# google-research/weatherbenchX

Hardware: AMD Instinct MI355X
Metric: grid-point·metric evals/s (0.25° 721×1440×37L) at 1/2/4/8 GPUs; % HBM roofline (higher is better)
Workload: dtype f32+f64

## Files before the change

### weatherbenchx_amd/csrc/wbx_common.hpp

```cpp
#pragma once
#include <hip/hip_runtime.h>

#include <cstdarg>
#include <cstdint>
#include <cstdio>
#include <cstring>

#include "../../include/wbx.h"

struct wbx_ctx {
  int device = 0;
  int num_cus = 256;
  hipStream_t stream = nullptr;
  bool own_stream = false;
  hipEvent_t ev_start = nullptr;
  hipEvent_t ev_stop = nullptr;
  void* fft_state = nullptr;
  void* s2_scratch = nullptr;
  size_t s2_scratch_size = 0;
  void* aidm_scratch = nullptr;
  size_t aidm_scratch_size = 0;
  void* atoms_clean = nullptr;
  void* patch_counters = nullptr;
  size_t patch_counters_size = 0;
  uint32_t ens_queue_parity = 0;
  hipEvent_t* marks = nullptr;
  int marks_used = 0, marks_made = 0, marks_cap = 0;
};

namespace wbx {

char* last_error_buf();

inline int fail(int code, const char* fmt, ...) {
  va_list ap;
  va_start(ap, fmt);
  vsnprintf(last_error_buf(), 512, fmt, ap);
  va_end(ap);
  return code;
}

template <typename T>
__device__ __forceinline__ T ld_stream(const T* p) {
#ifdef WBX_LD_STREAM_PLAIN
  return *p;
#else
  return __builtin_nontemporal_load(p);
#endif
}

__device__ __forceinline__ const char* uniform_ptr(const char* p) {
  const uint64_t v = (uint64_t)p;
  const uint32_t lo = __builtin_amdgcn_readfirstlane((uint32_t)v), hi = __builtin_amdgcn_readfirstlane((uint32_t)(v >> 32));
  return (const char*)(((uint64_t)hi << 32) | lo);
}

template <typename T>
using global_ptr = const __attribute__((address_space(1))) T*;

template <typename T>
using const_ptr = const __attribute__((address_space(4))) T*;

static __constant__ int64_t wbx_zero_i64[1] = {0};
static __constant__ double wbx_one_f64[1] = {1.0};

__device__ __forceinline__ int64_t readlane64(int64_t v, int j) {
  const int lo = __builtin_amdgcn_readlane((int)(uint32_t)(uint64_t)v, j);
  const int hi = __builtin_amdgcn_readlane((int)(uint32_t)((uint64_t)v >> 32), j);
  return (int64_t)(((uint64_t)(uint32_t)hi << 32) | (uint32_t)lo);
}

__device__ __forceinline__ double wave_sum(double v) {
#pragma unroll
  for (int o = 32; o > 0; o >>= 1) v += __shfl_xor(v, o, 64);
  return v;
}

template <int CTRL, int ROW_MASK>
__device__ __forceinline__ double dpp_moved(double v) {
  const int lo = __builtin_amdgcn_update_dpp(0, __double2loint(v), CTRL, ROW_MASK, 0xf, true);
  const int hi = __builtin_amdgcn_update_dpp(0, __double2hiint(v), CTRL, ROW_MASK, 0xf, true);
  return __hiloint2double(hi, lo);
}

__device__ __forceinline__ double wave_sum_lane63(double v) {
  v += dpp_moved<0xB1, 0xf>(v);
  v += dpp_moved<0x4E, 0xf>(v);
  v += dpp_moved<0x124, 0xf>(v);
  v += dpp_moved<0x128, 0xf>(v);
  v += dpp_moved<0x142, 0xa>(v);
  v += dpp_moved<0x143, 0xc>(v);
  return v;
}

__device__ __forceinline__ double wave_sum_uniform(double v) {
  const double t = wave_sum_lane63(v);
  return __hiloint2double(__builtin_amdgcn_readlane(__double2hiint(t), 63), __builtin_amdgcn_readlane(__double2loint(t), 63));
}

}

#define WBX_HIP(expr)                                                                   \
  do {                                                                                  \
    hipError_t _e = (expr);                                                             \
    if (_e != hipSuccess)                                                               \
      return wbx::fail(WBX_ERR_HIP, "%s failed: %s (%s:%d)", #expr, hipGetErrorString(_e), \
                       __FILE__, __LINE__);                                             \
  } while (0)

#define WBX_REQUIRE(cond, ...)                                   \
  do {                                                           \
    if (!(cond)) return wbx::fail(WBX_ERR_INVALID, __VA_ARGS__); \
  } while (0)
```

### weatherbenchx_amd/csrc/wbx_ctx.hip

```cpp
#include <cstdlib>

#include <set>

#include "wbx_common.hpp"

namespace wbx {
char* last_error_buf() {
  static thread_local char buf[512] = "";
  return buf;
}
}

extern "C" int wbx_abi_version(void) { return WBX_ABI_VERSION; }

extern "C" const char* wbx_last_error(void) { return wbx::last_error_buf(); }

extern "C" int wbx_device_count(int* n_out) {
  WBX_REQUIRE(n_out != nullptr, "n_out is NULL");
  int n = 0;
  hipError_t e = hipGetDeviceCount(&n);
  if (e != hipSuccess) {
    *n_out = 0;
    return wbx::fail(WBX_ERR_NO_DEVICE, "hipGetDeviceCount: %s", hipGetErrorString(e));
  }
  *n_out = n;
  return 0;
}

extern "C" int wbx_ctx_create(int device_id, void* hip_stream, wbx_ctx** out) {
  WBX_REQUIRE(out != nullptr, "out is NULL");
  *out = nullptr;
  int n = 0;
  if (hipGetDeviceCount(&n) != hipSuccess || n <= 0)
    return wbx::fail(WBX_ERR_NO_DEVICE, "no HIP device visible (libwbx_hip has no CPU path)");
  WBX_REQUIRE(device_id >= 0 && device_id < n, "device_id %d out of range [0,%d)", device_id, n);
  WBX_HIP(hipSetDevice(device_id));
  wbx_ctx* c = new wbx_ctx();
  c->device = device_id;
  int cus = 0;
  if (hipDeviceGetAttribute(&cus, hipDeviceAttributeMultiprocessorCount, device_id) == hipSuccess && cus > 0) c->num_cus = cus;
  if (hip_stream) {
    c->stream = reinterpret_cast<hipStream_t>(hip_stream);
    c->own_stream = false;
  } else {
    hipError_t e = hipStreamCreateWithFlags(&c->stream, hipStreamNonBlocking);
    if (e != hipSuccess) {
      delete c;
      return wbx::fail(WBX_ERR_HIP, "hipStreamCreate: %s", hipGetErrorString(e));
    }
    c->own_stream = true;
  }
  if (hipEventCreate(&c->ev_start) != hipSuccess || hipEventCreate(&c->ev_stop) != hipSuccess) {
    delete c;
    return wbx::fail(WBX_ERR_HIP, "hipEventCreate failed");
  }
  *out = c;
  return 0;
}

namespace wbx {
void spectrum_release(wbx_ctx* ctx);
void spectrum_note_write(const void* dst, size_t bytes);
}

extern "C" int wbx_ctx_destroy(wbx_ctx* ctx) {
  if (!ctx) return 0;
  (void)hipSetDevice(ctx->device);
  (void)hipStreamSynchronize(ctx->stream);
  wbx::spectrum_release(ctx);
  if (ctx->s2_scratch) (void)hipFree(ctx->s2_scratch);
  if (ctx->aidm_scratch) (void)hipFree(ctx->aidm_scratch);
  if (ctx->patch_counters) (void)hipFree(ctx->patch_counters);
  delete static_cast<std::set<const void*>*>(ctx->atoms_clean);
  if (ctx->ev_start) (void)hipEventDestroy(ctx->ev_start);
  if (ctx->ev_stop) (void)hipEventDestroy(ctx->ev_stop);
  for (int i = 0; i < ctx->marks_made; ++i) (void)hipEventDestroy(ctx->marks[i]);
  free(ctx->marks);
  if (ctx->own_stream && ctx->stream) (void)hipStreamDestroy(ctx->stream);
  delete ctx;
  return 0;
}

extern "C" int wbx_ctx_synchronize(wbx_ctx* ctx) {
  WBX_REQUIRE(ctx != nullptr, "ctx is NULL");
  WBX_HIP(hipStreamSynchronize(ctx->stream));
  return 0;
}

extern "C" int wbx_ctx_device_name(wbx_ctx* ctx, char* buf, size_t buflen) {
  WBX_REQUIRE(ctx != nullptr && buf != nullptr && buflen > 0, "bad arguments");
  hipDeviceProp_t prop;
  WBX_HIP(hipGetDeviceProperties(&prop, ctx->device));
  snprintf(buf, buflen, "%s|%s|cus=%d", prop.name, prop.gcnArchName, prop.multiProcessorCount);
  return 0;
}

extern "C" int wbx_malloc(wbx_ctx* ctx, size_t bytes, void** dptr_out) {
  WBX_REQUIRE(ctx != nullptr && dptr_out != nullptr, "bad arguments");
  *dptr_out = nullptr;
  if (bytes == 0) return 0;
  WBX_HIP(hipSetDevice(ctx->device));
  WBX_HIP(hipMalloc(dptr_out, bytes));
  return 0;
}

extern "C" int wbx_free(wbx_ctx* ctx, void* dptr) {
  WBX_REQUIRE(ctx != nullptr, "ctx is NULL");
  if (!dptr) return 0;
  WBX_HIP(hipSetDevice(ctx->device));
  WBX_HIP(hipStreamSynchronize(ctx->stream));
  {
    hipDeviceptr_t base = nullptr;
    size_t size = 0;
    if (hipMemGetAddressRange(&base, &size, dptr) != hipSuccess) {
      (void)hipGetLastError();
      size = 1;
    }
    wbx::spectrum_note_write(dptr, size);
  }
  WBX_HIP(hipFree(dptr));
  return 0;
}

extern "C" int wbx_memcpy_h2d(wbx_ctx* ctx, void* dptr, const void* h_src, size_t bytes) {
  WBX_REQUIRE(ctx != nullptr, "ctx is NULL");
  if (bytes == 0) return 0;
  WBX_REQUIRE(dptr != nullptr && h_src != nullptr, "NULL pointer");
  WBX_HIP(hipSetDevice(ctx->device));
  wbx::spectrum_note_write(dptr, bytes);
  WBX_HIP(hipMemcpyAsync(dptr, h_src, bytes, hipMemcpyHostToDevice, ctx->stream));
  WBX_HIP(hipStreamSynchronize(ctx->stream));
  return 0;
}

extern "C" int wbx_memcpy_d2h(wbx_ctx* ctx, void* h_dst, const void* dptr, size_t bytes) {
  WBX_REQUIRE(ctx != nullptr, "ctx is NULL");
  if (bytes == 0) return 0;
  WBX_REQUIRE(dptr != nullptr && h_dst != nullptr, "NULL pointer");
  WBX_HIP(hipSetDevice(ctx->device));
  WBX_HIP(hipMemcpyAsync(h_dst, dptr, bytes, hipMemcpyDeviceToHost, ctx->stream));
  WBX_HIP(hipStreamSynchronize(ctx->stream));
  return 0;
}

extern "C" int wbx_host_alloc(wbx_ctx* ctx, size_t bytes, void** h_out) {
  WBX_REQUIRE(ctx != nullptr && h_out != nullptr, "NULL argument");
  WBX_HIP(hipSetDevice(ctx->device));
  WBX_HIP(hipHostMalloc(h_out, bytes ? bytes : 8, hipHostMallocDefault));
  return 0;
}

extern "C" int wbx_host_free(wbx_ctx* ctx, void* h_ptr) {
  WBX_REQUIRE(ctx != nullptr, "ctx is NULL");
  if (h_ptr) WBX_HIP(hipHostFree(h_ptr));
  return 0;
}

extern "C" int wbx_memcpy_d2h_async(wbx_ctx* ctx, void* h_pinned, const void* dptr, size_t bytes) {
  WBX_REQUIRE(ctx != nullptr, "ctx is NULL");
  if (bytes == 0) return 0;
  WBX_REQUIRE(dptr != nullptr && h_pinned != nullptr, "NULL pointer");
  WBX_HIP(hipSetDevice(ctx->device));
  WBX_HIP(hipMemcpyAsync(h_pinned, dptr, bytes, hipMemcpyDeviceToHost, ctx->stream));
  return 0;
}

struct wbx_fence {
  hipEvent_t ev;
};

extern "C" int wbx_fence_create(wbx_ctx* ctx, wbx_fence** out) {
  WBX_REQUIRE(ctx != nullptr && out != nullptr, "NULL argument");
  WBX_HIP(hipSetDevice(ctx->device));
  wbx_fence* f = new wbx_fence;
  hipError_t e = hipEventCreateWithFlags(&f->ev, hipEventDisableTiming);
  if (e != hipSuccess) {
    delete f;
    WBX_HIP(e);
  }
  *out = f;
  return 0;
}

extern "C" int wbx_fence_record(wbx_ctx* ctx, wbx_fence* f) {
  WBX_REQUIRE(ctx != nullptr && f != nullptr, "NULL argument");
  WBX_HIP(hipEventRecord(f->ev, ctx->stream));
  return 0;
}

extern "C" int wbx_fence_wait(wbx_fence* f) {
  WBX_REQUIRE(f != nullptr, "fence is NULL");
  WBX_HIP(hipEventSynchronize(f->ev));
  return 0;
}

extern "C" int wbx_ctx_wait_fence(wbx_ctx* ctx, wbx_fence* f) {
  WBX_REQUIRE(ctx != nullptr && f != nullptr, "NULL argument");
  WBX_HIP(hipStreamWaitEvent(ctx->stream, f->ev, 0));
  return 0;
}

extern "C" int wbx_fence_destroy(wbx_fence* f) {
  if (f) {
    (void)hipEventDestroy(f->ev);
    delete f;
  }
  return 0;
}

extern "C" int wbx_memset(wbx_ctx* ctx, void* dptr, int value, size_t bytes) {
  WBX_REQUIRE(ctx != nullptr, "ctx is NULL");
  if (bytes == 0) return 0;
  WBX_REQUIRE(dptr != nullptr, "NULL pointer");
  wbx::spectrum_note_write(dptr, bytes);
  WBX_HIP(hipMemsetAsync(dptr, value, bytes, ctx->stream));
  return 0;
}

extern "C" int wbx_timer_start(wbx_ctx* ctx) {
  WBX_REQUIRE(ctx != nullptr, "ctx is NULL");
  WBX_HIP(hipEventRecord(ctx->ev_start, ctx->stream));
  return 0;
}

extern "C" int wbx_mark(wbx_ctx* ctx, int* index_out) {
  WBX_REQUIRE(ctx != nullptr && index_out != nullptr, "bad arguments");
// ... 77 lines not shown
```

### weatherbenchx_amd/csrc/wbx_ens.hip

```cpp
#include "wbx_ens_atoms.hpp"
#include "wbx_ens_impl.hpp"

namespace wbx {

static int ens_common(wbx_ctx* ctx, const wbx_s1_plan* plan, int dtype, int M, int64_t member_stride, int algo,
                      const void* p, const void* t, const uint8_t* mask, double* out, bool map, int lane) {
  WBX_REQUIRE(ctx != nullptr, "ctx is NULL");
  if (int rc = check_plan(plan)) return rc;
  WBX_REQUIRE(plan->vec == 1, "ensemble kernels use vec=1");
  if (plan->flags & WBX_FLAG_MASKED) WBX_REQUIRE(mask != nullptr, "WBX_FLAG_MASKED set but mask is NULL");
  WBX_REQUIRE(M >= 1, "ensemble size must be >= 1 (got %d)", M);
  WBX_REQUIRE(algo == WBX_ENS_SORT || algo == WBX_ENS_PAIRWISE || (algo == WBX_ENS_DIAG_LOADONLY && (M == 50 || M == 51)) ||
                  (algo == WBX_ENS_DIAG_PAIRWISE_LDS && M == 51),
              "unknown ensemble algorithm %d", algo);
  const bool empty = plan->nkey * plan->ndepth * plan->nx == 0;
  WBX_REQUIRE(empty || (p != nullptr && t != nullptr), "predictions/targets pointer is NULL");
  WBX_REQUIRE(out != nullptr || plan->nkey == 0, "output pointer is NULL");
  WBX_HIP(hipSetDevice(ctx->device));
  S1Args a;
  fill_args(plan, a);
  a.in[0] = p;
  a.in[1] = t;
  a.in[3] = mask;
  a.out = out;
  a.M = M;
  a.mstride = member_stride;
  a.lane = lane;
  if (dtype == WBX_F64) return launch_ens_op<EnsOpGeneric<double>>(ctx, plan, a, map);
  WBX_REQUIRE(dtype == WBX_F32, "unknown dtype %d", dtype);
  if (plan->flags & WBX_FLAG_SKIPNA_ENS) {
    static const bool generic = getenv("WBX_ENS_SKIPNA_GENERIC") && atoi(getenv("WBX_ENS_SKIPNA_GENERIC")) != 0;
    if (generic || M > 64) return launch_ens_op<EnsOpGeneric<float>>(ctx, plan, a, map);
    algo = WBX_ENS_SKIPNA_SORT;
  }
  if (M == 51) return launch_ens_m51(ctx, plan, a, algo, map);
  if (M == 50) return launch_ens_m50(ctx, plan, a, algo, map);
  if (M <= 4) return launch_ens_m4(ctx, plan, a, algo, map);
  if (M <= 8) return launch_ens_m8(ctx, plan, a, algo, map);
  if (M <= 16) return launch_ens_m16(ctx, plan, a, algo, map);
  if (M <= 32) return launch_ens_m32(ctx, plan, a, algo, map);
  if (M <= 64) return launch_ens_m64(ctx, plan, a, algo, map);
  return launch_ens_op<EnsOpGeneric<float>>(ctx, plan, a, map);
}

}

extern "C" int wbx_ens_partial(wbx_ctx* ctx, const wbx_s1_plan* plan, int dtype, int M, int64_t member_stride,
                               int algo, const void* p, const void* t, const uint8_t* mask, double* partial_out) {
  return wbx::ens_common(ctx, plan, dtype, M, member_stride, algo, p, t, mask, partial_out, false, 0);
}

extern "C" int wbx_ens_map(wbx_ctx* ctx, const wbx_s1_plan* plan, int dtype, int M, int64_t member_stride, int algo,
                           int lane, const void* p, const void* t, double* out) {
  if (lane < 0 || lane >= WBX_ENS_LANES) return wbx::fail(WBX_ERR_INVALID, "ensemble lane %d out of range", lane);
  return wbx::ens_common(ctx, plan, dtype, M, member_stride, algo, p, t, nullptr, out, true, lane);
}

namespace wbx {

static int ens_binned_geometry(const wbx_s1_plan* plan, int64_t nA, int64_t nBk, int64_t nBr, int32_t w_on_x, BinnedArgs& g) {
  if (int rc = check_plan(plan)) return rc;
  WBX_REQUIRE(nA >= 1 && nBk >= 1 && nBr >= 1 && plan->nx >= 1 && plan->ndepth >= 1, "empty geometry");
  patch_geometry(g, nA * nBk, nBk, nBr, (w_on_x & WBX_BINNED_W_ON_X) ? plan->nx : 1, plan->ndepth, plan->nx, ens_atoms_rows(), ens_atoms_taper());
  return 0;
}

}

extern "C" int wbx_ens_binned_atoms_size(const wbx_s1_plan* plan, int64_t nA, int64_t nBk, int64_t nBr, int32_t w_on_x,
                                         int64_t* bytes_out) {
  using namespace wbx;
  WBX_REQUIRE(bytes_out != nullptr, "bytes_out is NULL");
  BinnedArgs g;
  if (int rc = ens_binned_geometry(plan, nA, nBk, nBr, w_on_x, g)) return rc;
  *bytes_out = (int64_t)atoms_carve(g, nullptr);
  return 0;
}

extern "C" int wbx_ens_binned_atoms(wbx_ctx* ctx, const wbx_s1_plan* plan, int64_t nA, int64_t nBk, int64_t nBr,
                                    int32_t w_on_x, const uint64_t* bits, void* atoms_out, int64_t* overflow_out) {
  using namespace wbx;
  WBX_REQUIRE(ctx != nullptr, "ctx is NULL");
  WBX_REQUIRE(bits != nullptr && atoms_out != nullptr, "NULL pointer");
  BinnedArgs g;
  if (int rc = ens_binned_geometry(plan, nA, nBk, nBr, w_on_x, g)) return rc;
  WBX_HIP(hipSetDevice(ctx->device));
  atoms_carve(g, atoms_out);
  if (int rc = atoms_launch(ctx, g, bits, plan->ndepth, plan->nx, true)) return rc;
  if (overflow_out) {
    const size_t n = (size_t)g.nBk * g.nrs * g.nxt;
    int32_t* host = (int32_t*)malloc(n * sizeof(int32_t));
    WBX_REQUIRE(host != nullptr, "out of host memory");
    hipError_t err = hipMemcpyAsync(host, g.nwords, n * sizeof(int32_t), hipMemcpyDeviceToHost, ctx->stream);
    if (err == hipSuccess) err = hipStreamSynchronize(ctx->stream);
    int64_t bad = 0;
    for (size_t i = 0; i < n && err == hipSuccess; ++i) bad += host[i] < 0;
    free(host);
    WBX_HIP(err);
    *overflow_out = bad;
  }
  return 0;
}

extern "C" int wbx_ens_binned(wbx_ctx* ctx, const wbx_s1_plan* plan, int dtype, int M, int64_t member_stride, int algo,
                              const void* p, const void* t, const uint8_t* mask, const double* wt, const uint64_t* bits,
                              int64_t nA, int64_t nBk, int64_t nBr, int32_t w_on_x, int32_t nbin, const void* atoms,
                              double* out) {
  using namespace wbx;
  WBX_REQUIRE(ctx != nullptr, "ctx is NULL");
  if (int rc = check_plan(plan)) return rc;
  WBX_REQUIRE(dtype == WBX_F32, "wbx_ens_binned takes float32 members (got dtype %d)", dtype);
  WBX_REQUIRE(algo == WBX_ENS_SORT, "wbx_ens_binned runs the rank form (WBX_ENS_SORT) only");
  WBX_REQUIRE(M >= 2 && M <= 64, "wbx_ens_binned handles 2..64 members (got %d)", M);
  WBX_REQUIRE(!(plan->flags & WBX_FLAG_SKIPNA_ENS), "wbx_ens_binned does not take skipna_ensemble (per-point member counts)");
  WBX_REQUIRE(nbin >= 1 && nbin <= 64, "wbx_ens_binned handles 1..64 bins (got %d)", nbin);
  WBX_REQUIRE(nA >= 0 && nBk >= 0 && nBr >= 0 && nA * nBk * nBr == plan->nkey, "nA*nBk*nBr must equal plan->nkey");
  WBX_REQUIRE((w_on_x & ~63) == 0 && (w_on_x & 6) != 6, "w_on_x: unknown or contradictory WBX_BINNED_* flags (%d)", w_on_x);
  WBX_REQUIRE(wt == nullptr || (w_on_x & (WBX_BINNED_WT_X_ONLY | WBX_BINNED_WT_ROW_ONLY)),
              "wbx_ens_binned takes factored weights only (WBX_BINNED_WT_X_ONLY / WBX_BINNED_WT_ROW_ONLY), or wt = NULL");
  WBX_REQUIRE(!(w_on_x & WBX_BINNED_WT_X_ONLY) || (w_on_x & WBX_BINNED_W_ON_X), "WBX_BINNED_WT_X_ONLY needs WBX_BINNED_W_ON_X");
  const bool twin_out = (plan->flags & WBX_FLAG_MASKED) && (w_on_x & WBX_BINNED_TWIN_MASK);
  const bool skipna = (plan->flags & WBX_FLAG_SKIPNA) != 0;
  const int64_t nout = nA * nBk * (skipna ? (twin_out ? 20 : 10) : (twin_out ? ENS_ATOMS_NOUT2 : ENS_ATOMS_NOUT)) * nbin;
  if (nout == 0) return 0;
  WBX_REQUIRE(out != nullptr, "out is NULL");
  WBX_HIP(hipSetDevice(ctx->device));
  if (nBr * plan->ndepth * plan->nx == 0) {
    if (!(w_on_x & WBX_BINNED_ACCUMULATE)) WBX_HIP(hipMemsetAsync(out, 0, (size_t)nout * sizeof(double), ctx->stream));
    return 0;
  }
  WBX_REQUIRE(p != nullptr && t != nullptr && bits != nullptr, "p/t/bits is NULL");
  if (plan->flags & WBX_FLAG_MASKED) {
    WBX_REQUIRE(mask != nullptr, "WBX_FLAG_MASKED set but mask is NULL");
    WBX_REQUIRE(w_on_x & WBX_BINNED_W_ON_X, "wbx_ens_binned with a validity mask needs W indexed per x (WBX_BINNED_W_ON_X)");
    WBX_REQUIRE(plan->xstride[3] >= 0, "the mask's x stride must be non-negative");
  }
  WBX_REQUIRE(plan->xstride[0] >= 0 && plan->xstride[1] >= 0 && (double)plan->nx * (double)plan->xstride[0] * 4.0 < 4294967296.0 &&
                  (double)plan->nx * (double)plan->xstride[1] * 4.0 < 4294967296.0,
              "x offsets of the members and of the targets must be non-negative and fit 32 bits");
  S1Args a;
  fill_args(plan, a);
  a.in[0] = p;
  a.in[1] = t;
  a.in[3] = mask;
  a.M = M;
  a.mstride = member_stride;
  EnsBinnedCall c;
  c.wt = wt;
  c.bits = bits;
  c.nA = nA;
  c.nBk = nBk;
  c.nBr = nBr;
  c.nj = (w_on_x & WBX_BINNED_W_ON_X) ? plan->nx : 1;
  c.nbin = nbin;
  c.w_on_x = w_on_x;
  c.prepared = atoms;
  c.out = out;
  if (M == 51) return launch_ens_atoms_m51(ctx, plan, a, c);
  if (M == 50) return launch_ens_atoms_m50(ctx, plan, a, c);
  if (M <= 4) return launch_ens_atoms_m4(ctx, plan, a, c);
  if (M <= 8) return launch_ens_atoms_m8(ctx, plan, a, c);
  if (M <= 16) return launch_ens_atoms_m16(ctx, plan, a, c);
  if (M <= 32) return launch_ens_atoms_m32(ctx, plan, a, c);
  return launch_ens_atoms_m64(ctx, plan, a, c);
}
```

### weatherbenchx_amd/csrc/wbx_ens_impl.hpp

```cpp
#pragma once
#include <cmath>
#include <cstdlib>

#include "wbx_s1.hpp"
#include "wbx_sortnet_gen.hpp"
#include "wbx_sortnet3_gen.hpp"

#ifndef WBX_ENS_MIN_WAVES
#define WBX_ENS_MIN_WAVES 1
#endif

#ifndef WBX_ENS_MIN_WAVES_PLAIN
#define WBX_ENS_MIN_WAVES_PLAIN WBX_ENS_MIN_WAVES
#endif
#ifndef WBX_ENS_SORTNET3
#define WBX_ENS_SORTNET3 1
#endif

#ifndef WBX_ENS_NOFALLBACK
#define WBX_ENS_NOFALLBACK 0
#endif
#ifndef WBX_ENS_STATS32
#define WBX_ENS_STATS32 1
#endif

namespace wbx {

constexpr int WBX_ENS_DIAG_LOADONLY = 99;
constexpr int WBX_ENS_DIAG_PAIRWISE_LDS = 98;
constexpr int WBX_ENS_SKIPNA_SORT = 97;

template <typename T>
struct EnsOpGeneric {
  static constexpr int NIN = 2;
  static constexpr int NLANE = WBX_ENS_LANES;
  static constexpr int NACC = WBX_ENS_LANES;
  static constexpr int XR_UNROLL = 1, XK_UNROLL = 1, MIN_WAVES = 1;

  __device__ __forceinline__ static void values(const S1Args& a, const int64_t (&ro)[WBX_MAX_INPUTS], int64_t x,
                                                double (&val)[NLANE]) {
    const int M = a.M;
    const T* pp = reinterpret_cast<const T*>(a.in[0]) + ro[0] + x * a.xstride[0];
    const double td = (double)(reinterpret_cast<const T*>(a.in[1])[ro[1] + x * a.xstride[1]]);
    const bool skip = a.flags & WBX_FLAG_SKIPNA_ENS;
    double se = 0.0, sq = 0.0, sabs = 0.0, pair_total = 0.0, x0 = 0.0;
    int n = 0;
    for (int i = 0; i < M; ++i) {
      const double xi = (double)pp[(int64_t)i * a.mstride];
      if (skip && xi != xi) continue;
      if (n == 0) x0 = xi;
      ++n;
      const double e = xi - x0;
      se += e;
      sq = fma(e, e, sq);
      sabs += fabs(xi - td);
      double row = 0.0;
      for (int j = 0; j < i; ++j) {
        const double xj = (double)pp[(int64_t)j * a.mstride];
        if (skip && xj != xj) continue;
        row += fabs(xi - xj);
      }
      pair_total += row;
    }
    const double dM = (double)n;
    const double fair = (a.flags & WBX_FLAG_FAIR) ? 1.0 : 0.0;
    const double mean_e = se / dM;
    const double mean_d = (x0 - td) + mean_e;
    const double var = (sq - se * mean_e) / (dM - 1.0);
    val[0] = sabs / dM;
    val[1] = 2.0 * pair_total / (dM * (dM - fair));
    val[2] = var;
    val[3] = mean_d * mean_d - var / dM;
    val[4] = mean_d * mean_d;
  }

  template <int V, bool XK>
  __device__ __forceinline__ static void accum(const S1Args& a, const int64_t (&ro)[WBX_MAX_INPUTS], int64_t x,
                                               double (&acc)[XK ? V : 1][NACC]) {
    static_assert(V == 1, "ensemble op is one point per lane");
    double val[NLANE];
    values(a, ro, x, val);
#pragma unroll
    for (int l = 0; l < NLANE; ++l) acc[0][l] += val[l];
  }
};

template <int MP, bool EXACT, int ALGO>
struct EnsOpF32 {
  static constexpr int NIN = 2;
  static constexpr int NLANE = WBX_ENS_LANES;
  static constexpr int NACC = WBX_ENS_LANES;
  static constexpr int XR_UNROLL = 1, XK_UNROLL = 1, MIN_WAVES = WBX_ENS_MIN_WAVES_PLAIN;

  struct Regs {
    float xm[MP];
    float t;
    float poison;
  };

  __device__ __forceinline__ static void load(const S1Args& a, const int64_t (&ro)[WBX_MAX_INPUTS], int64_t x, Regs& r) {
    const int M = EXACT ? MP : a.M;
    const float* pp = reinterpret_cast<const float*>(a.in[0]) + ro[0] + x * a.xstride[0];
    r.t = ld_stream(reinterpret_cast<const float*>(a.in[1]) + ro[1] + x * a.xstride[1]);
#pragma unroll
    for (int m = 0; m < MP; ++m) r.xm[m] = (EXACT || m < M) ? ld_stream(pp + (int64_t)m * a.mstride) : INFINITY;
  }

  __device__ __forceinline__ static void values(const S1Args& a, const int64_t (&ro)[WBX_MAX_INPUTS], int64_t x,
                                                double (&val)[NLANE]) {
    Regs r;
    load(a, ro, x, r);
    finish(a, ro, x, r, val);
  }

  template <bool FAST32 = false>
  __device__ __forceinline__ static bool compute(const S1Args& a, Regs& r, double (&val)[NLANE]) {
    const int M = EXACT ? MP : a.M;
    const double td = (double)r.t;
    float(&xm)[MP] = r.xm;

    if constexpr (ALGO == WBX_ENS_DIAG_LOADONLY) {
      float s = 0.f;
#pragma unroll
      for (int m = 0; m < MP; ++m)
        if (EXACT || m < M) s += xm[m];
      val[0] = (double)s - td;
      val[1] = val[2] = val[3] = val[4] = 0.0;
      return false;
    }
    double pair_total = 0.0;
    float poison = 0.f;
    int nvalid = 0;
    bool weird = false;
    float shift32 = 0.f;
    if constexpr (ALGO == WBX_ENS_SKIPNA_SORT) {
      const bool tfin32 = (r.t - r.t) == 0.f;
      shift32 = r.t;
      if (__builtin_amdgcn_ballot_w64(!tfin32)) {
        float lo = INFINITY;
#pragma unroll
        for (int m = 0; m < MP; ++m)
          if (EXACT || m < M) lo = fminf(lo, xm[m]);
        shift32 = tfin32 ? r.t : lo;
      }
#pragma unroll
      for (int m = 0; m < MP; ++m) {
        if (EXACT || m < M) {
          const float x = xm[m];
          const bool missing = x != x;
          nvalid += missing ? 0 : 1;
          xm[m] = missing ? shift32 : x;
        }
      }
      if constexpr (!EXACT) {
        float big = 0.f;
        int m = 0;
// ... 168 lines not shown
    const double mean_d = x0t + mean_e;
    const double var = (sq - se * mean_e) * inv_m1;
    double spread;
    if constexpr (ALGO == WBX_ENS_SORT) {
      spread = dot * spread_scale;
    } else {
      spread = pair_total * spread_scale;
    }
    if constexpr (ALGO == WBX_ENS_DIAG_PAIRWISE_LDS) {
      static_assert(EXACT && MP % 17 == 0, "the LDS-tiled diagnostic is instantiated for M = 51");
      constexpr int B = 17, NB = MP / B;
      __shared__ float tile[MP][64];
      float* col = &tile[0][threadIdx.x];
#pragma unroll
      for (int m = 0; m < MP; ++m) col[m * 64] = xm[m];
      asm volatile("" ::: "memory");
      double total = 0.0;
#pragma unroll
      for (int bi = 0; bi < NB; ++bi) {
        float xi[B];
#pragma unroll
        for (int k = 0; k < B; ++k) xi[k] = col[(bi * B + k) * 64];
#pragma unroll
        for (int k = 1; k < B; ++k) {
          float row = 0.f;
#pragma unroll
          for (int l = 0; l < k; ++l) row += fabsf(xi[k] - xi[l]);
          total += (double)row;
        }
#pragma unroll
        for (int bj = 0; bj < bi; ++bj) {
          float xj[B];
#pragma unroll
          for (int l = 0; l < B; ++l) xj[l] = col[(bj * B + l) * 64];
#pragma unroll
          for (int k = 0; k < B; ++k) {
            float row = 0.f;
#pragma unroll
            for (int l = 0; l < B; ++l) row += fabsf(xi[k] - xj[l]);
            total += (double)row;
          }
        }
      }
      spread = total * spread_scale;
    }
    val[0] = sabs * inv_m;
    val[1] = spread;
    val[2] = var;
    val[3] = mean_d * mean_d - var * inv_m;
    val[4] = mean_d * mean_d;
  }

  __device__ __forceinline__ static void stats32(const S1Args& a, float (&xm)[MP], const float t, const float poison,
                                                 double (&val)[NLANE]) {
    static_assert(EXACT, "fp32 chain sums are instantiated for the exact-M buckets");
    constexpr int K = 8, MID = MP / 2, NPAIR = MP / 2;
    const float c = xm[MID];
    float se[K], sq[K], sa[K], dt[K];
#pragma unroll
    for (int k = 0; k < K; ++k) se[k] = sq[k] = sa[k] = dt[k] = k == 0 ? poison : 0.f;
#pragma unroll
    for (int i = 0; i < NPAIR; ++i) {
      const int j = MP - 1 - i, k = i % K;
      const float ei = xm[i] - c, ej = xm[j] - c;
      se[k] += ei + ej;
      sq[k] = fmaf(ei, ei, sq[k]);
      sq[k] = fmaf(ej, ej, sq[k]);
      sa[k] += fabsf(xm[i] - t);
      sa[k] += fabsf(xm[j] - t);
      dt[k] = fmaf((float)(MP - 1 - 2 * i), xm[j] - xm[i], dt[k]);
    }
    if constexpr (MP & 1) {
      sa[NPAIR % K] += fabsf(c - t);
    } else {
    }
    auto fold = [](const float (&v)[K]) {
      return ((double)(v[0] + v[4]) + (double)(v[1] + v[5])) + ((double)(v[2] + v[6]) + (double)(v[3] + v[7]));
    };
    const double dse = fold(se), dsq = fold(sq), dsa = fold(sa), ddt = fold(dt);
    constexpr double dM = (double)MP;
    const double fair = (a.flags & WBX_FLAG_FAIR) ? 1.0 : 0.0;
    constexpr double inv_m = 1.0 / dM, inv_m1 = 1.0 / (dM - 1.0);
    const double spread_scale = 2.0 / (dM * (dM - fair));
    const double mean_e = dse * inv_m;
    const double mean_d = ((double)c - (double)t) + mean_e;
    const double var = (dsq - dse * mean_e) * inv_m1;
    val[0] = dsa * inv_m;
    val[1] = ddt * spread_scale;
    val[2] = var;
    val[3] = mean_d * mean_d - var * inv_m;
    val[4] = mean_d * mean_d;
  }

  template <int V, bool XK>
  __device__ __forceinline__ static void accum(const S1Args& a, const int64_t (&ro)[WBX_MAX_INPUTS], int64_t x,
                                               double (&acc)[XK ? V : 1][NACC]) {
    static_assert(V == 1, "ensemble op is one point per lane");
    double val[NLANE];
    values(a, ro, x, val);
#pragma unroll
    for (int l = 0; l < NLANE; ++l) acc[0][l] += val[l];
  }
};

template <class Core, bool SKIPNA>
struct EnsMasked {
  static constexpr int NIN = Core::NIN;
  static constexpr int NLANE = Core::NLANE;
  static constexpr int NACC = Core::NLANE + (SKIPNA ? Core::NLANE : 1);
  static constexpr int XR_UNROLL = 1, XK_UNROLL = 1, MIN_WAVES = WBX_ENS_MIN_WAVES;

  __device__ __forceinline__ static void values(const S1Args& a, const int64_t (&ro)[WBX_MAX_INPUTS], int64_t x,
                                                double (&val)[NLANE]) {
    Core::values(a, ro, x, val);
  }

  template <int V, bool XK>
  __device__ __forceinline__ static void accum(const S1Args& a, const int64_t (&ro)[WBX_MAX_INPUTS], int64_t x,
                                               double (&acc)[XK ? V : 1][NACC]) {
    static_assert(V == 1, "ensemble op is one point per lane");
    double val[NLANE];
    Core::values(a, ro, x, val);
    const bool valid =
        (a.flags & WBX_FLAG_MASKED) ? reinterpret_cast<const uint8_t*>(a.in[3])[ro[3] + x * a.xstride[3]] != 0 : true;
    if constexpr (!SKIPNA) {
#pragma unroll
      for (int l = 0; l < NLANE; ++l) acc[0][l] += valid ? val[l] : 0.0;
      acc[0][NLANE] += valid ? 1.0 : 0.0;
    } else {
#pragma unroll
      for (int l = 0; l < NLANE; ++l) {
        const bool ok = valid && !(val[l] != val[l]);
        acc[0][l] += ok ? val[l] : 0.0;
        acc[0][NLANE + l] += ok ? 1.0 : 0.0;
      }
    }
  }
};


#pragma clang diagnostic push
#pragma clang diagnostic ignored "-Winline-asm"
#ifndef WBX_ENS_PIPE_NLDS
#define WBX_ENS_PIPE_NLDS 50
#endif
#ifndef WBX_ENS_PIPE_WAVES
#define WBX_ENS_PIPE_WAVES 3
#endif
#ifndef WBX_ENS_PIPE_SKIPNA_WAVES
#define WBX_ENS_PIPE_SKIPNA_WAVES 3
#endif
template <int MP, bool EXACT, int ALGO, bool FLAT>
__global__ void __launch_bounds__(64, ALGO == WBX_ENS_SKIPNA_SORT ? WBX_ENS_PIPE_SKIPNA_WAVES : WBX_ENS_PIPE_WAVES)
ens_pipe_kernel(S1Args a, int R) {
  using Op = EnsOpF32<MP, EXACT, ALGO>;
  constexpr int NA = Op::NACC;
  constexpr int NLDS = MP < WBX_ENS_PIPE_NLDS ? MP : WBX_ENS_PIPE_NLDS;
  constexpr int NREG = MP - NLDS;
  __shared__ float stage[NLDS][64];
  const int lane = threadIdx.x;
  const int M = EXACT ? MP : a.M;
  const int64_t b = blockIdx.x;
  const int64_t key = b / a.nchunk;
  const int chunk = (int)(b - key * a.nchunk);
  const int64_t d0 = (int64_t)chunk * a.dchunk;
  const int64_t d1 = d0 + a.dchunk < a.D ? d0 + a.dchunk : a.D;
  const int nx = (int)a.nx;
  const uint32_t lds0 = (uint32_t)(uintptr_t)(__attribute__((address_space(3))) void*)&stage[0][0];
  const int64_t mstride_b = a.mstride * 4;

  int64_t kb[WBX_MAX_INPUTS], ro[WBX_MAX_INPUTS];
  key_bases<2>(a, key, kb);
  double acc[NA];
#pragma unroll
  for (int l = 0; l < NA; ++l) acc[l] = 0.0;

  int64_t d = d0, e0 = 0, e1 = 0, et = 0;
  int wm = 0;
  const int wstep = 64 % nx;
  auto open_segment = [&]() {
    if constexpr (FLAT) {
      const int64_t plane = d / R;
      const int64_t j0 = d - plane * R;
      const int64_t nj = d1 - d < R - j0 ? d1 - d : R - j0;
      row_bases<2>(a, kb, key, plane * R, ro);
      e0 = j0 * nx;
      e1 = (j0 + nj) * nx;
      et = e0 & ~(int64_t)63;
      wm = (int)((et + lane) % nx);
      d += nj;
    } else {
      row_bases<2>(a, kb, key, d, ro);
      e0 = 0;
      e1 = nx;
      et = 0;
      d += 1;
    }
  };

  float xn[NREG > 0 ? NREG : 1], tn = 0.f;
  double wn = 0.0;
  auto issue = [&]() {
    int64_t e = et + lane;
    e = e < e0 ? e0 : (e < e1 ? e : e1 - 1);
    const uint32_t voff = (uint32_t)e * (uint32_t)a.xstride[0] * 4u;
    const char* um = uniform_ptr(reinterpret_cast<const char*>(a.in[0]) + ro[0] * 4);
#pragma unroll
    for (int m = 0; m < NLDS; ++m) {
      if (EXACT || m < M)
        asm volatile("s_add_u32 m0, %2, %3\n\tglobal_load_lds_dword %0, %1 nt" ::"v"(voff), "s"(um), "s"(lds0), "i"(m * 256)
                     : "memory", "scc", "m0");
      um += mstride_b;
      asm volatile("" : "+s"(um));
    }
    const float* pr = reinterpret_cast<const float*>(a.in[0]) + ro[0] + e * a.xstride[0];
#pragma unroll
    for (int m = NLDS; m < MP; ++m) xn[m - NLDS] = (EXACT || m < M) ? ld_stream(pr + (int64_t)m * a.mstride) : INFINITY;
    tn = ld_stream(reinterpret_cast<const float*>(a.in[1]) + ro[1] + e * a.xstride[1]);
    if constexpr (FLAT) wn = a.xw[wm];
  };

  bool more = d < d1;
  if (more) {
    open_segment();
    issue();
  }
  while (more) {
    typename Op::Regs r;
    asm volatile("s_waitcnt vmcnt(0)" ::: "memory");
#pragma unroll
    for (int m = 0; m < NLDS; ++m) r.xm[m] = (EXACT || m < M) ? stage[m][lane] : INFINITY;
#pragma unroll
    for (int m = NLDS; m < MP; ++m) r.xm[m] = xn[m - NLDS];
    r.t = tn;
    const double wcur = wn;
    const int64_t ecur = et + lane;
    const bool valid = ecur >= e0 && ecur < e1;
    const int64_t xcur = ecur < e0 ? e0 : (ecur < e1 ? ecur : e1 - 1);
    int64_t rocur[WBX_MAX_INPUTS];
#pragma unroll
    for (int i = 0; i < WBX_MAX_INPUTS; ++i) rocur[i] = ro[i];
    const bool full = et >= e0 && et + 64 <= e1;
    et += 64;
    if (et >= e1) {
      more = d < d1;
      if (more) open_segment();
    } else if constexpr (FLAT) {
      wm += wstep;
      wm = wm >= nx ? wm - nx : wm;
    }
    asm volatile("s_waitcnt lgkmcnt(0)" ::: "memory");
    if (more) issue();
    double val[Op::NLANE];
    Op::template finish<true>(a, rocur, xcur, r, val);
    if constexpr (FLAT) {
      if (full) {
#pragma unroll
        for (int l = 0; l < NA; ++l) acc[l] = fma(val[l], wcur, acc[l]);
      } else {
#pragma unroll
        for (int l = 0; l < NA; ++l) acc[l] = fma(valid ? val[l] : 0.0, wcur, acc[l]);
      }
    } else if (full) {
#pragma unroll
      for (int l = 0; l < NA; ++l) acc[l] += val[l];
    } else {
#pragma unroll
      for (int l = 0; l < NA; ++l) acc[l] += valid ? val[l] : 0.0;
    }
  }
#pragma unroll
  for (int l = 0; l < NA; ++l) {
    const double v = wave_sum(acc[l]);
    if (lane == l) a.out[(key * a.nchunk + chunk) * NA + l] = v;
  }
}

#pragma clang diagnostic pop

inline bool ens_pipe_ok(const wbx_s1_plan* plan, const S1Args& a, bool skipna_ens = false) {
  static const bool off = getenv("WBX_ENS_PIPE") && atoi(getenv("WBX_ENS_PIPE")) == 0;
  static const bool off_skipna = getenv("WBX_ENS_PIPE_SKIPNA") && atoi(getenv("WBX_ENS_PIPE_SKIPNA")) == 0;
  if (off || (skipna_ens && off_skipna)) return false;
  if (plan->x_kept || plan->x_weights != nullptr || plan->block_threads != 64) return false;
  if (plan->flags & (WBX_FLAG_MASKED | WBX_FLAG_SKIPNA | (skipna_ens ? 0u : (unsigned)WBX_FLAG_SKIPNA_ENS))) return false;
  if (plan->nx <= 0 || plan->ndepth <= 0 || plan->nkey <= 0) return false;
  if (a.xstride[0] < 0 || a.xstride[1] < 0) return false;
  return (double)plan->nx * (double)a.xstride[0] * 4.0 < 4294967296.0;
}

inline bool ens_pipe_flat_ok(const wbx_s1_plan* plan, const S1Args& a) {
  static const bool off = getenv("WBX_ENS_PIPE") && atoi(getenv("WBX_ENS_PIPE")) == 0;
  if (off) return false;
  if (plan->x_kept || plan->x_weights == nullptr || plan->block_threads != 64 || plan->plane_rows <= 0) return false;
  if (plan->flags & (WBX_FLAG_MASKED | WBX_FLAG_SKIPNA | WBX_FLAG_SKIPNA_ENS)) return false;
  if (plan->nx <= 0 || plan->nx > WBX_XW_MAX || plan->ndepth <= 0 || plan->nkey <= 0 || plan->ndepth % plan->plane_rows != 0) return false;
  if (a.xstride[0] != 1 || a.xstride[1] != 1) return false;
  return (double)plan->nx * (double)plan->plane_rows * 4.0 < 4294967296.0;
}

template <int MP, bool EXACT, int ALGO, bool FLAT = false>
int launch_ens_pipe(wbx_ctx* ctx, const wbx_s1_plan* plan, S1Args& a) {
  const int64_t grid = plan->nkey * plan->nchunk;
  WBX_REQUIRE(grid < (int64_t)1 << 31, "grid too large (%lld blocks)", (long long)grid);
  hipLaunchKernelGGL((ens_pipe_kernel<MP, EXACT, ALGO, FLAT>), dim3((unsigned)grid), dim3(64), 0, ctx->stream, a,
                     FLAT ? plan->plane_rows : 0);
  WBX_HIP(hipGetLastError());
  return 0;
}

template <class Op>
int launch_ens_op(wbx_ctx* ctx, const wbx_s1_plan* plan, S1Args& a, bool map) {
  if (map) return launch_map<Op>(ctx, plan, a);
  if (plan->x_weights != nullptr) {
    WBX_REQUIRE(!(plan->flags & WBX_FLAG_SKIPNA_ENS), "flat x-weighted mode does not take skipna_ensemble");
    if (plan->flags & WBX_FLAG_SKIPNA) return launch_flat_weighted1<EnsMasked<Op, true>>(ctx, plan, a);
    if (plan->flags & WBX_FLAG_MASKED) return launch_flat_weighted1<EnsMasked<Op, false>>(ctx, plan, a);
    return launch_flat_weighted1<Op>(ctx, plan, a);
  }
  if (plan->flags & WBX_FLAG_SKIPNA) return launch_partial<EnsMasked<Op, true>, 1>(ctx, plan, a);
  if (plan->flags & WBX_FLAG_MASKED) return launch_partial<EnsMasked<Op, false>, 1>(ctx, plan, a);
  return launch_partial<Op, 1>(ctx, plan, a);
}

template <int MP, bool EXACT>
int launch_ens_bucket(wbx_ctx* ctx, const wbx_s1_plan* plan, S1Args& a, int algo, bool map) {
  if (!map && algo == WBX_ENS_SORT && ens_pipe_ok(plan, a)) return launch_ens_pipe<MP, EXACT, WBX_ENS_SORT>(ctx, plan, a);
  if (!map && algo == WBX_ENS_SORT && ens_pipe_flat_ok(plan, a)) return launch_ens_pipe<MP, EXACT, WBX_ENS_SORT, true>(ctx, plan, a);
  if (algo == WBX_ENS_SORT) return launch_ens_op<EnsOpF32<MP, EXACT, WBX_ENS_SORT>>(ctx, plan, a, map);
  if (algo == WBX_ENS_DIAG_LOADONLY) {
    if (!EXACT || map) return fail(WBX_ERR_INVALID, "the load-only diagnostic exists for the exact-M partial kernels only");
    return launch_partial<EnsOpF32<MP, EXACT, WBX_ENS_DIAG_LOADONLY>, 1>(ctx, plan, a);
  }
  if (algo == WBX_ENS_DIAG_PAIRWISE_LDS) {
    if constexpr (EXACT && MP == 51) {
      if (map || plan->x_weights != nullptr || (plan->flags & (WBX_FLAG_MASKED | WBX_FLAG_SKIPNA)) || plan->block_threads != 64)
        return fail(WBX_ERR_INVALID, "the LDS-tiled pair-form diagnostic exists for the plain partial kernels with one-wave blocks only");
      return launch_partial<EnsOpF32<MP, EXACT, WBX_ENS_DIAG_PAIRWISE_LDS>, 1>(ctx, plan, a);
    } else {
      return fail(WBX_ERR_INVALID, "the LDS-tiled pair-form diagnostic exists for M = 51 only");
    }
  }
  if (!map && algo == WBX_ENS_SKIPNA_SORT && ens_pipe_ok(plan, a, true)) return launch_ens_pipe<MP, EXACT, WBX_ENS_SKIPNA_SORT>(ctx, plan, a);
  if (algo == WBX_ENS_SKIPNA_SORT) return launch_ens_op<EnsOpF32<MP, EXACT, WBX_ENS_SKIPNA_SORT>>(ctx, plan, a, map);
  return launch_ens_op<EnsOpF32<MP, EXACT, WBX_ENS_PAIRWISE>>(ctx, plan, a, map);
}

int launch_ens_m4(wbx_ctx*, const wbx_s1_plan*, S1Args&, int, bool);
int launch_ens_m8(wbx_ctx*, const wbx_s1_plan*, S1Args&, int, bool);
int launch_ens_m16(wbx_ctx*, const wbx_s1_plan*, S1Args&, int, bool);
int launch_ens_m32(wbx_ctx*, const wbx_s1_plan*, S1Args&, int, bool);
int launch_ens_m64(wbx_ctx*, const wbx_s1_plan*, S1Args&, int, bool);
int launch_ens_m50(wbx_ctx*, const wbx_s1_plan*, S1Args&, int, bool);
int launch_ens_m51(wbx_ctx*, const wbx_s1_plan*, S1Args&, int, bool);

}
```

Measured before the change: 119.5 billion.

## Taper tail of ensemble pipe grid by splitting last blocks into pieces

Splits the final logical blocks of the ensemble pipe kernel into 2/4/8 sub-pieces sized from the number of blocks that can be resident at once. Each piece covers a slice of the tile range and writes a partial sum to scratch, and a small fixup kernel then adds the partials into the output. The goal is to cut the tail-wave imbalance where a few long blocks run alone at the end of the launch. The cost is an extra kernel launch, scratch traffic, occupancy queries cached per kernel, and extra index arithmetic in every block.

```diff
diff --git a/weatherbenchx_amd/csrc/wbx_common.hpp b/weatherbenchx_amd/csrc/wbx_common.hpp
--- a/weatherbenchx_amd/csrc/wbx_common.hpp
+++ b/weatherbenchx_amd/csrc/wbx_common.hpp
@@ -24,6 +24,10 @@
   void* patch_counters = nullptr;
   size_t patch_counters_size = 0;
   uint32_t ens_queue_parity = 0;
+  void* ens_taper_scratch = nullptr;
+  size_t ens_taper_scratch_size = 0;
+  int32_t ens_pipe_last[5] = {0, 0, 0, 0, 0};
+  void* ens_pipe_resident = nullptr;
   hipEvent_t* marks = nullptr;
   int marks_used = 0, marks_made = 0, marks_cap = 0;
 };
diff --git a/weatherbenchx_amd/csrc/wbx_ctx.hip b/weatherbenchx_amd/csrc/wbx_ctx.hip
--- a/weatherbenchx_amd/csrc/wbx_ctx.hip
+++ b/weatherbenchx_amd/csrc/wbx_ctx.hip
@@ -1,5 +1,6 @@
 #include <cstdlib>
 
+#include <map>
 #include <set>
 
 #include "wbx_common.hpp"
@@ -71,7 +72,9 @@
   if (ctx->s2_scratch) (void)hipFree(ctx->s2_scratch);
   if (ctx->aidm_scratch) (void)hipFree(ctx->aidm_scratch);
   if (ctx->patch_counters) (void)hipFree(ctx->patch_counters);
+  if (ctx->ens_taper_scratch) (void)hipFree(ctx->ens_taper_scratch);
   delete static_cast<std::set<const void*>*>(ctx->atoms_clean);
+  delete static_cast<std::map<const void*, int>*>(ctx->ens_pipe_resident);
   if (ctx->ev_start) (void)hipEventDestroy(ctx->ev_start);
   if (ctx->ev_stop) (void)hipEventDestroy(ctx->ev_stop);
   for (int i = 0; i < ctx->marks_made; ++i) (void)hipEventDestroy(ctx->marks[i]);
diff --git a/weatherbenchx_amd/csrc/wbx_ens.hip b/weatherbenchx_amd/csrc/wbx_ens.hip
--- a/weatherbenchx_amd/csrc/wbx_ens.hip
+++ b/weatherbenchx_amd/csrc/wbx_ens.hip
@@ -164,3 +164,37 @@
   if (M <= 32) return launch_ens_atoms_m32(ctx, plan, a, c);
   return launch_ens_atoms_m64(ctx, plan, a, c);
 }
+
+extern "C" int wbx_test_ens_taper_plan(int64_t N, int64_t G, int64_t Tmax, const int32_t* tiers16, int32_t* geom_out) {
+  WBX_REQUIRE(tiers16 != nullptr && geom_out != nullptr, "NULL pointer");
+  const int32_t tiers[3] = {tiers16[0], tiers16[1], tiers16[2]};
+  const wbx::EnsPipeTaper t = wbx::ens_taper_plan(N, G, Tmax, tiers);
+  geom_out[0] = t.nwhole;
+  for (int k = 0; k < 3; ++k) geom_out[1 + k] = t.cnt[k];
+  return 0;
+}
+
+extern "C" int wbx_test_ens_taper_piece(const int32_t* geom, int32_t block, int32_t T, int32_t* piece_out) {
+  WBX_REQUIRE(geom != nullptr && piece_out != nullptr, "NULL pointer");
+  wbx::EnsPipeTaper t{};
+  t.nwhole = geom[0];
+  for (int k = 0; k < 3; ++k) t.cnt[k] = geom[1 + k];
+  WBX_REQUIRE(block >= t.nwhole && block - t.nwhole < wbx::ens_taper_pieces(t), "block %d is not a piece", (int)block);
+  int32_t lb, j, s, t0, t1, first, s2;
+  wbx::ens_taper_piece(t, block - t.nwhole, lb, j, s);
+  wbx::ens_taper_tiles(T, j, s, t0, t1);
+  wbx::ens_taper_row(t, lb - t.nwhole, first, s2);
+  WBX_REQUIRE(s == s2 && first + j == block - t.nwhole, "piece and row arithmetic disagree at block %d", (int)block);
+  piece_out[0] = lb;
+  piece_out[1] = t0;
+  piece_out[2] = t1;
+  piece_out[3] = first;
+  piece_out[4] = 1 << s;
+  return 0;
+}
+
+extern "C" int wbx_test_ens_pipe_last_launch(wbx_ctx* ctx, int32_t* last_out) {
+  WBX_REQUIRE(ctx != nullptr && last_out != nullptr, "NULL pointer");
+  for (int k = 0; k < 5; ++k) last_out[k] = ctx->ens_pipe_last[k];
+  return 0;
+}
diff --git a/weatherbenchx_amd/csrc/wbx_ens_impl.hpp b/weatherbenchx_amd/csrc/wbx_ens_impl.hpp
--- a/weatherbenchx_amd/csrc/wbx_ens_impl.hpp
+++ b/weatherbenchx_amd/csrc/wbx_ens_impl.hpp
@@ -1,7 +1,10 @@
 #pragma once
 #include <cmath>
+#include <cstdio>
 #include <cstdlib>
-
+#include <map>
+
+#include "wbx_ens_taper.hpp"
 #include "wbx_s1.hpp"
 #include "wbx_sortnet_gen.hpp"
 #include "wbx_sortnet3_gen.hpp"
@@ -476,7 +479,7 @@
 #endif
 template <int MP, bool EXACT, int ALGO, bool FLAT>
 __global__ void __launch_bounds__(64, ALGO == WBX_ENS_SKIPNA_SORT ? WBX_ENS_PIPE_SKIPNA_WAVES : WBX_ENS_PIPE_WAVES)
-ens_pipe_kernel(S1Args a, int R) {
+ens_pipe_kernel(S1Args a, int R, EnsPipeTaper tp) {
   using Op = EnsOpF32<MP, EXACT, ALGO>;
   constexpr int NA = Op::NACC;
   constexpr int NLDS = MP < WBX_ENS_PIPE_NLDS ? MP : WBX_ENS_PIPE_NLDS;
@@ -484,12 +487,34 @@
   __shared__ float stage[NLDS][64];
   const int lane = threadIdx.x;
   const int M = EXACT ? MP : a.M;
-  const int64_t b = blockIdx.x;
+  const bool piece = !FLAT && (int)blockIdx.x >= tp.nwhole;
+  int32_t lb = (int32_t)blockIdx.x, pj = 0, ps = 0;
+  if constexpr (!FLAT) {
+    if (piece) ens_taper_piece(tp, (int32_t)blockIdx.x - tp.nwhole, lb, pj, ps);
+  }
+  const int64_t b = lb;
   const int64_t key = b / a.nchunk;
   const int chunk = (int)(b - key * a.nchunk);
-  const int64_t d0 = (int64_t)chunk * a.dchunk;
-  const int64_t d1 = d0 + a.dchunk < a.D ? d0 + a.dchunk : a.D;
   const int nx = (int)a.nx;
+  int64_t d0 = (int64_t)chunk * a.dchunk;
+  int64_t d1 = d0 + a.dchunk < a.D ? d0 + a.dchunk : a.D;
+  int32_t efirst = 0, elast = nx;
+  if constexpr (!FLAT) {
+    if (piece) {
+      int32_t t0, t1;
+      ens_taper_tiles((int32_t)(d1 - d0) * tp.tpr, pj, ps, t0, t1);
+      if (t0 < t1) {
+        const int32_t r0 = (int32_t)((uint32_t)t0 / (uint32_t)tp.tpr), r1 = (int32_t)((uint32_t)(t1 - 1) / (uint32_t)tp.tpr);
+        efirst = (t0 - r0 * tp.tpr) * 64;
+        elast = (t1 - r1 * tp.tpr) * 64;
+        elast = elast < nx ? elast : nx;
+        d1 = d0 + r1 + 1;
+        d0 += r0;
+      } else {
+        d1 = d0;
+      }
+    }
+  }
   const uint32_t lds0 = (uint32_t)(uintptr_t)(__attribute__((address_space(3))) void*)&stage[0][0];
   const int64_t mstride_b = a.mstride * 4;
 
@@ -516,9 +541,9 @@
     } else {
       row_bases<2>(a, kb, key, d, ro);
       e0 = 0;
-      e1 = nx;
       et = 0;
       d += 1;
+      e1 = d == d1 ? elast : nx;
     }
   };
 
@@ -547,6 +572,7 @@
   bool more = d < d1;
   if (more) {
     open_segment();
+    if constexpr (!FLAT) et = efirst;
     issue();
   }
   while (more) {
@@ -593,11 +619,25 @@
       for (int l = 0; l < NA; ++l) acc[l] += valid ? val[l] : 0.0;
     }
   }
+  double* const dst = piece ? tp.scratch + (int64_t)((int32_t)blockIdx.x - tp.nwhole) * NA : a.out + (key * a.nchunk + chunk) * NA;
 #pragma unroll
   for (int l = 0; l < NA; ++l) {
     const double v = wave_sum(acc[l]);
-    if (lane == l) a.out[(key * a.nchunk + chunk) * NA + l] = v;
-  }
+    if (lane == l) dst[l] = v;
+  }
+}
+
+template <int NA>
+__global__ void __launch_bounds__(256) ens_pipe_fixup_kernel(EnsPipeTaper tp, double* __restrict__ out) {
+  const int32_t idx = (int32_t)(blockIdx.x * 256 + threadIdx.x);
+  if (idx >= ens_taper_rows(tp) * NA) return;
+  const int32_t i = idx / NA, l = idx - i * NA;
+  int32_t first, s;
+  ens_taper_row(tp, i, first, s);
+  const double* src = tp.scratch + (int64_t)first * NA + l;
+  double v = src[0];
+  for (int32_t j = 1; j < (1 << s); ++j) v += src[(int64_t)j * NA];
+  out[((int64_t)tp.nwhole + i) * NA + l] = v;
 }
 
 #pragma clang diagnostic pop
@@ -623,13 +663,70 @@
   return (double)plan->nx * (double)plan->plane_rows * 4.0 < 4294967296.0;
 }
 
+#ifndef WBX_ENS_PIPE_TAPER_TIERS
+#define WBX_ENS_PIPE_TAPER_TIERS {8, 4, 2}
+#endif
+inline int ens_pipe_taper_setup(wbx_ctx* ctx, const void* kernel, const wbx_s1_plan* plan, int NA, EnsPipeTaper& tp) {
+  ctx->ens_pipe_last[0] = tp.nwhole;
+  for (int k = 1; k < 5; ++k) ctx->ens_pipe_last[k] = 0;
+  const char* on = getenv("WBX_ENS_PIPE_TAPER");
+  if (on && atoi(on) == 0) return 0;
+  int32_t tiers16[3] = WBX_ENS_PIPE_TAPER_TIERS;
+  if (const char* spec = getenv("WBX_ENS_PIPE_TAPER_TIERS")) {
+    int v[3] = {0, 0, 0};
+    WBX_REQUIRE(sscanf(spec, "%d,%d,%d", &v[0], &v[1], &v[2]) == 3 && v[0] >= 0 && v[1] >= 0 && v[2] >= 0 && v[0] + v[1] + v[2] <= 1024,
+                "WBX_ENS_PIPE_TAPER_TIERS='%s': three counts of logical blocks in sixteenths of the resident blocks", spec);
+    for (int k = 0; k < 3; ++k) tiers16[k] = v[k];
+  }
+  auto* occ = static_cast<std::map<const void*, int>*>(ctx->ens_pipe_resident);
+  if (!occ) ctx->ens_pipe_resident = occ = new std::map<const void*, int>();
+  auto it = occ->find(kernel);
+  if (it == occ->end()) {
+    int per_cu = 0;
+    WBX_HIP(hipOccupancyMaxActiveBlocksPerMultiprocessor(&per_cu, kernel, 64, 0));
+    it = occ->emplace(kernel, per_cu * ctx->num_cus).first;
+  }
+  const int64_t nlb = plan->nkey * plan->nchunk, tpr = (plan->nx + 63) / 64;
+  EnsPipeTaper t = ens_taper_plan(nlb, it->second, plan->depth_chunk * tpr, tiers16);
+  ctx->ens_pipe_last[0] = t.nwhole;
+  for (int k = 0; k < 3; ++k) ctx->ens_pipe_last[1 + k] = t.cnt[k];
+  ctx->ens_pipe_last[4] = it->second;
+  if (ens_taper_rows(t) == 0) return 0;
+  const size_t need = (size_t)ens_taper_pieces(t) * NA * sizeof(double);
+  if (ctx->ens_taper_scratch_size < need) {
+    if (ctx->ens_taper_scratch) {
+      WBX_HIP(hipStreamSynchronize(ctx->stream));
+      WBX_HIP(hipFree(ctx->ens_taper_scratch));
+      ctx->ens_taper_scratch = nullptr;
+      ctx->ens_taper_scratch_size = 0;
+    }
+    WBX_HIP(hipMalloc(&ctx->ens_taper_scratch, need));
+    ctx->ens_taper_scratch_size = need;
+  }
+  t.tpr = (int32_t)tpr;
+  t.scratch = reinterpret_cast<double*>(ctx->ens_taper_scratch);
+  tp = t;
+  return 0;
+}
+
 template <int MP, bool EXACT, int ALGO, bool FLAT = false>
 int launch_ens_pipe(wbx_ctx* ctx, const wbx_s1_plan* plan, S1Args& a) {
-  const int64_t grid = plan->nkey * plan->nchunk;
-  WBX_REQUIRE(grid < (int64_t)1 << 31, "grid too large (%lld blocks)", (long long)grid);
-  hipLaunchKernelGGL((ens_pipe_kernel<MP, EXACT, ALGO, FLAT>), dim3((unsigned)grid), dim3(64), 0, ctx->stream, a,
-                     FLAT ? plan->plane_rows : 0);
+  const int64_t nlb = plan->nkey * plan->nchunk;
+  WBX_REQUIRE(nlb < (int64_t)1 << 31, "grid too large (%lld blocks)", (long long)nlb);
+  constexpr int NA = EnsOpF32<MP, EXACT, ALGO>::NACC;
+  const auto kernel = ens_pipe_kernel<MP, EXACT, ALGO, FLAT>;
+  EnsPipeTaper tp{};
+  tp.nwhole = (int32_t)nlb;
+  if constexpr (!FLAT) {
+    if (int rc = ens_pipe_taper_setup(ctx, reinterpret_cast<const void*>(kernel), plan, NA, tp)) return rc;
+  }
+  const int64_t grid = (int64_t)tp.nwhole + ens_taper_pieces(tp);
+  hipLaunchKernelGGL(kernel, dim3((unsigned)grid), dim3(64), 0, ctx->stream, a, FLAT ? plan->plane_rows : 0, tp);
   WBX_HIP(hipGetLastError());
+  if (const int32_t rows = ens_taper_rows(tp)) {
+    hipLaunchKernelGGL(ens_pipe_fixup_kernel<NA>, dim3((unsigned)((rows * NA + 255) / 256)), dim3(256), 0, ctx->stream, tp, a.out);
+    WBX_HIP(hipGetLastError());
+  }
   return 0;
 }
 
diff --git a/weatherbenchx_amd/csrc/wbx_ens_taper.hpp b/weatherbenchx_amd/csrc/wbx_ens_taper.hpp
--- /dev/null
+++ b/weatherbenchx_amd/csrc/wbx_ens_taper.hpp
@@ -0,0 +1,59 @@
+#pragma once
+#include <cstdint>
+
+#if defined(__HIPCC__)
+#include <hip/hip_runtime.h>
+#define WBX_HD __host__ __device__ __forceinline__
+#else
+#define WBX_HD inline
+#endif
+
+namespace wbx {
+
+struct EnsPipeTaper {
+  int32_t nwhole;
+  int32_t cnt[3];
+  int32_t tpr;
+  double* scratch;
+};
+
+WBX_HD int32_t ens_taper_rows(const EnsPipeTaper& t) { return t.cnt[0] + t.cnt[1] + t.cnt[2]; }
+WBX_HD int32_t ens_taper_pieces(const EnsPipeTaper& t) { return 2 * t.cnt[0] + 4 * t.cnt[1] + 8 * t.cnt[2]; }
+
+WBX_HD void ens_taper_piece(const EnsPipeTaper& t, int32_t p, int32_t& lb, int32_t& j, int32_t& s) {
+  const int32_t o1 = 2 * t.cnt[0], o2 = o1 + 4 * t.cnt[1];
+  s = p < o1 ? 1 : (p < o2 ? 2 : 3);
+  const int32_t q = p - (p < o1 ? 0 : (p < o2 ? o1 : o2));
+  lb = t.nwhole + (p < o1 ? 0 : (p < o2 ? t.cnt[0] : t.cnt[0] + t.cnt[1])) + (q >> s);
+  j = q & ((1 << s) - 1);
+}
+
+WBX_HD void ens_taper_row(const EnsPipeTaper& t, int32_t i, int32_t& first, int32_t& s) {
+  const int32_t c0 = t.cnt[0], c1 = t.cnt[1];
+  s = i < c0 ? 1 : (i < c0 + c1 ? 2 : 3);
+  first = i < c0 ? 2 * i : (i < c0 + c1 ? 2 * c0 + 4 * (i - c0) : 2 * c0 + 4 * c1 + 8 * (i - c0 - c1));
+}
+
+WBX_HD void ens_taper_tiles(int32_t T, int32_t j, int32_t s, int32_t& t0, int32_t& t1) {
+  const int32_t P = 1 << s;
+  t0 = (j * T + P - 1) >> s;
+  t1 = ((j + 1) * T + P - 1) >> s;
+}
+
+inline EnsPipeTaper ens_taper_plan(int64_t N, int64_t G, int64_t Tmax, const int32_t (&tiers16)[3]) {
+  EnsPipeTaper t{};
+  t.nwhole = (int32_t)N;
+  if (G <= 0 || N < G || Tmax >= ((int64_t)1 << 27)) return t;
+  int64_t c[3];
+  for (int k = 0; k < 3; ++k) c[k] = (tiers16[k] > 0 && Tmax >= ((int64_t)2 << k)) ? G * tiers16[k] / 16 : 0;
+  for (int k = 0; k < 3; ++k) {
+    const int64_t over = c[0] + c[1] + c[2] - N;
+    if (over > 0) c[k] = c[k] > over ? c[k] - over : 0;
+  }
+  if (N - c[0] - c[1] - c[2] + 2 * c[0] + 4 * c[1] + 8 * c[2] >= ((int64_t)1 << 31)) return t;
+  for (int k = 0; k < 3; ++k) t.cnt[k] = (int32_t)c[k];
+  t.nwhole = (int32_t)(N - c[0] - c[1] - c[2]);
+  return t;
+}
+
+}
```

New measurement: 119.7 billion (median of 2 runs). No clear change (+0.1%).
